# yvokeller/Show-Attend-and-Tell

Hardware: AMD Instinct MI355X
Metric: train images/sec on COCO batch=128 at 1/2/4/8 MI355X (higher is better)
Workload: dtype bf16; 1 GPU; COCO-shaped resnet152 encoder (bf16 fwd) + attention/tf/ado decoder train step, V=10000, T=27; global_batch=128, per_gpu_batch=128, seq_len=27, parallelism=dp1, hip_graph=True, encoder_decoder_overlap=True

## Files before the change

### show-attend-and-tell_amd/csrc/decoder.hip

```cpp
#include "sat_common.h"
#include "sat_internal.h"

namespace {

struct WS {
  float *mean_f, *hc0, *hc0pre, *xg, *gctx_const, *hg, *gctx, *uh_all, *gates_all, *c_in, *c_out, *h_out, *ctx_all,
      *gate_all, *fh, *fz;
  void *mean_t, *Ws, *emb_t, *h_in_t, *ctx_t, *gated_t, *hd_t, *comb_t;
  int32_t* tok;
  uint8_t* dmask;
  void *dpre_t, *dfh_t, *dfz_t, *dhg_t, *dWs_t, *dpre0_t;
  float *dcomb, *dhd, *dctx_head, *dhg, *dgated, *dh_rec, *dc, *dWs_acc, *dv_acc, *dbv_acc, *part, *demb, *dpre0,
      *colsum, *de_all;
  unsigned* ticket;
  float* gsplit;
  unsigned* gtickets;
  float* xt;
  float* fzp;
  float* am_val;
  int32_t* am_idx;
  void* emb_ws;
};
constexpr int kTicketBlocks = 16;

// ... 154 lines not shown
}

struct FGWS {
  float *dctx, *addend, *mean_term;
};
size_t carve_fg(const SatDecoderDims& d, char* base, FGWS* w) {
  const size_t B = d.B, L = d.L, D = d.D, R = B * (d.T - 1), f = 4;
  Carver c{base};
  c.take(w->dctx, R * D * f);
  if (d.attention) c.take(w->addend, B * L * D * f);
  else w->addend = nullptr;
  c.take(w->mean_term, B * D * f);
  return c.off + 256;
}

__global__ void start_tokens_kernel(int32_t* tok, int B, int T1, int start) {
  int b = blockIdx.x * blockDim.x + threadIdx.x;
  if (b < B) tok[(long)b * T1] = start;
}

__global__ void tf_prefill_kernel(const int64_t* __restrict__ caps, int B, int T, int V, int start,
                                  const uint8_t* __restrict__ keep_in, float p, const float* __restrict__ p_dev,
                                  uint64_t seed, const uint64_t* __restrict__ seed_ptr, int32_t* __restrict__ pre,
                                  uint8_t* __restrict__ keep_out) {
  const int T1 = T - 1;
  const int i = blockIdx.x * blockDim.x + threadIdx.x;
  if (i >= B * T1) return;
  const int b = i / T1, t = i - b * T1;
  bool keep = true;
  int tok = start;
  if (t > 0) {
    const int64_t c = caps[(long)b * T + t];
    tok = (c < 0 || c >= V) ? 0 : (int)c;
    if (keep_in) {
      keep = keep_in[i] != 0;
    } else {
      if (seed_ptr) seed ^= *seed_ptr * 0xD1B54A32D192ED03ULL;
      keep = sat_tf_uniform(seed, b, t) < (p_dev ? *p_dev : p);
    }
  }
  pre[i] = keep ? tok : -1;
  if (keep_out) keep_out[i] = keep ? 1 : 0;
}

struct Sampled {
  const int64_t* captions;
  float p; const float* p_dev;
  const uint8_t* mask; uint8_t* mask_out;
};
inline int32_t* tok_pre(const WS& w) { return (int32_t*)w.demb; }

template <typename T>
__global__ void ado_combine_rows_kernel(const float* fh, const float* fz, const T* emb, int rows, int E, long ld,
                                        T* comb) {
  const long n = (long)rows * E;
  for (long i = blockIdx.x * (long)blockDim.x + threadIdx.x; i < n; i += (long)gridDim.x * blockDim.x) {
    const long r = i / E;
    const int e = (int)(i - r * E);
    const long o = r * ld + e;
    comb[o] = (T)(fh[o] + fz[o] + (float)emb[o]);
  }
}

int combine_rows(const float* fh, const float* fz, const void* emb, int rows, int E, long ld, int dtype, void* comb,
                 hipStream_t s) {
  long n = (long)rows * E;
  int g = (int)((n + 255) / 256);
  if (g > 4096) g = 4096;
  if (dtype == SAT_BF16)
    hipLaunchKernelGGL(ado_combine_rows_kernel<bf16>, dim3(g), dim3(256), 0, s, fh, fz, (const bf16*)emb, rows, E, ld, (bf16*)comb);
  else
    hipLaunchKernelGGL(ado_combine_rows_kernel<float>, dim3(g), dim3(256), 0, s, fh, fz, (const float*)emb, rows, E, ld, (float*)comb);
  return (int)hipGetLastError();
}

template <typename T>
__global__ void init_state_kernel(const float* pre, int splits, long stride, int B, int E, float* hc0, T* h_t,
                                  long h_ld, float* c_in, long c_ld) {
  const long n = (long)B * 2 * E;
  for (long i = blockIdx.x * (long)blockDim.x + threadIdx.x; i < n; i += (long)gridDim.x * blockDim.x) {
    const int b = (int)(i / (2 * E)), j = (int)(i - (long)b * 2 * E);
    const float v = tanhf(sum_parts(pre, i, splits, stride));
    hc0[i] = v;
    if (j < E) h_t[(long)b * h_ld + j] = (T)v;
    else c_in[(long)b * c_ld + j - E] = v;
  }
}

struct Ctx {
  SatDecoderDims d;
  SatDecoderLayout lay;
  const float* P;
  const void* LP;
  int ts;
  long T1, R, HG;
  bool tr;
  const void* W(int64_t off) const {
    return d.dtype == SAT_BF16 ? (const void*)((const bf16*)LP + off) : (const void*)(P + off);
  }
  const float* F(int64_t off) const { return P + off; }
  void* at(void* p, long elems) const { return (char*)p + elems * ts; }
  const void* at(const void* p, long elems) const { return (const char*)p + elems * ts; }
};

int linear(const Ctx& c, int rows, int N, int K, const void* x, long ldx, const void* w, long ldw, const float* bias,
           void* y, long ldy, int y_dtype, int act, hipStream_t s, const void* add1 = nullptr, long ld_add1 = 0,
           int add1_dtype = SAT_F32, void* aux = nullptr, long ld_aux = 0, int aux_dtype = SAT_F32,
           int splits = 0, long split_stride = 0) {
  SatGemm g;
  g.partial_splits = splits; g.split_stride = split_stride;
  g.M = rows; g.N = N; g.K = K; g.dtype = c.d.dtype;
  g.A = x; g.lda = ldx; g.B = w; g.ldb = ldw;
  g.C = y; g.ldc = ldy; g.c_dtype = y_dtype; g.bias = bias; g.act = act;
  g.add1 = add1; g.ld_add1 = ld_add1; g.add1_dtype = add1_dtype;
  g.aux = aux; g.ld_aux = ld_aux; g.aux_dtype = aux_dtype;
  return sat_gemm_launch(g, s);
}

int head_forward(const Ctx& c, const WS& w, int rows, int t, bool per_step, void* preds, const uint8_t* mask_in,
                 hipStream_t s) {
  const SatDecoderDims& d = c.d;
  const int E = d.E, D = d.D, V = d.V;
  const long rs = per_step ? c.T1 : 1;
  const long oE = per_step ? (long)t * E : 0, oD = per_step ? (long)t * D : 0, oV = per_step ? (long)t * V : 0;
  if (per_step)
    SAT_CHECK((hipError_t)sat_dropout_apply(w.h_out + oE, c.T1 * E, d.B, 1, E, d.training, d.has_dropout_mask,
                                            mask_in ? mask_in + oE : nullptr, w.dmask + oE, c.T1 * E, d.seed,
                                            d.seed_ptr, t,
                                            c.at(w.hd_t, oE), c.T1 * E, d.dtype, s));
  else
    SAT_CHECK((hipError_t)sat_dropout_apply(w.h_out, E, d.B, (int)c.T1, E, d.training, d.has_dropout_mask, mask_in,
                                            w.dmask, E, d.seed, d.seed_ptr, 0, w.hd_t, E, d.dtype, s));
  if (d.ado) {
    SAT_CHECK((hipError_t)linear(c, rows, E, E, c.at(w.hd_t, oE), rs * E, c.W(c.lay.fh_w), E, c.F(c.lay.fh_b),
                                 w.fh + oE, rs * E, SAT_F32, SAT_ACT_RELU, s));
    SAT_CHECK((hipError_t)linear(c, rows, E, D, c.at(w.ctx_t, oD), rs * D, c.W(c.lay.fz_w), D, c.F(c.lay.fz_b),
                                 w.fz + oE, rs * E, SAT_F32, SAT_ACT_RELU, s));
    SAT_CHECK((hipError_t)combine_rows(w.fh + oE, w.fz + oE, c.at(w.emb_t, oE), rows, E, rs * E, d.dtype,
                                       c.at(w.comb_t, oE), s));
    SAT_CHECK((hipError_t)linear(c, rows, V, E, c.at(w.comb_t, oE), rs * E, c.W(c.lay.fout_w), E,
                                 c.F(c.lay.fout_b), c.at(preds, oV), rs * V, d.dtype, SAT_ACT_RELU, s));
  } else {
    SAT_CHECK((hipError_t)linear(c, rows, V, E, c.at(w.hd_t, oE), rs * E, c.W(c.lay.do_w), E, c.F(c.lay.do_b),
                                 c.at(preds, oV), rs * V, d.dtype, SAT_ACT_NONE, s));
  }
  return 0;
}

struct StepIO {
  const void* feats;
  float* alphas;
  const float* d_alphas;
};

int fwd_hgemm(const Ctx& c, const WS& w, const Splits& sp, int t, hipStream_t s) {
  const SatDecoderDims& d = c.d;
  const int B = d.B, D = d.D, E = d.E;
  const long T1 = c.T1, HG = c.HG;
  const void* h_t = c.at(w.h_in_t, (long)t * E);
  if (d.attention)
    return linear(c, B, (int)HG, E, h_t, T1 * E, c.W(c.lay.hcat_w), E, c.F(c.lay.hcat_b), w.hg, HG, SAT_F32,
                  SAT_ACT_NONE, s, nullptr, 0, SAT_F32, nullptr, 0, SAT_F32, sp.h, (long)B * HG);
  return linear(c, B, 4 * E, E, h_t, T1 * E, c.W(c.lay.hcat_w + (long)(E + D) * E), E, c.F(c.lay.hcat_b + E + D),
                w.hg + E + D, HG, SAT_F32, SAT_ACT_NONE, s, nullptr, 0, SAT_F32, nullptr, 0, SAT_F32, sp.h,
                (long)B * HG);
}

int fwd_attn(const Ctx& c, const WS& w, const Splits& sp, const StepIO& io, int t, hipStream_t s) {
  const SatDecoderDims& d = c.d;
  const int B = d.B, L = d.L, D = d.D, E = d.E;
  const long T1 = c.T1, HG = c.HG;
  AttnFwdArgs a{};
  a.B = B; a.L = L; a.D = D; a.E = E; a.dtype = d.dtype;
  a.Ws = w.Ws; a.uh = w.hg; a.uh_ld = HG; a.v_w = c.F(c.lay.v_w); a.v_b = c.F(c.lay.v_b); a.a = io.feats;
  a.gate_pre = w.hg + E; a.gate_ld = HG;
  a.hg_splits = sp.h; a.hg_split_stride = (long)B * HG;
  a.alpha = io.alphas + (long)t * L; a.alpha_ld = T1 * L;
  a.ctx = w.ctx_all + (long)t * D; a.ctx_ld = T1 * D;
  a.ctx_t = c.at(w.ctx_t, (long)t * D); a.ctx_t_ld = T1 * D;
  a.gate = w.gate_all + (long)t * D; a.gate_out_ld = T1 * D;
  a.gated = c.at(w.gated_t, (long)t * D); a.gated_ld = T1 * D;
  a.uh_save = w.uh_all + (long)t * E; a.uh_save_ld = T1 * E;
  return sat_attention_fwd_launch(a, s);
}

int fwd_cgemm(const Ctx& c, const WS& w, const Splits& sp, int t, hipStream_t s) {
  const SatDecoderDims& d = c.d;
  const int B = d.B, D = d.D, E = d.E;
  return linear(c, B, 4 * E, D, c.at(w.gated_t, (long)t * D), c.T1 * D, c.W(c.lay.wih + E), E + D, nullptr, w.gctx,
                4 * E, SAT_F32, SAT_ACT_NONE, s, nullptr, 0, SAT_F32, nullptr, 0, SAT_F32, sp.c, (long)B * 4 * E);
}

// ... 375 lines not shown
                         (long)B * 2 * E, B, E, w.hc0, (float*)w.h_in_t, (long)T1 * E, w.c_in, (long)T1 * E);
    SAT_LAUNCH_CHECK();
  }
  if (att) {
    SAT_CHECK((hipError_t)linear(c, B * L, E, D, img_features, D, c.W(lay->attW_w), D, c.F(lay->attW_b), w.Ws, E,
                                 d.dtype, SAT_ACT_NONE, s));
  } else {
    SAT_CHECK((hipError_t)linear(c, B, 4 * E, D, w.mean_t, D, c.W(lay->wih + E), E + D, nullptr, w.gctx_const, 4 * E,
                                 SAT_F32, SAT_ACT_NONE, s));
    SAT_CHECK((hipError_t)sat_broadcast_rows(w.mean_t, B, D, T1, d.dtype, w.gated_t, s));
    SAT_CHECK((hipError_t)sat_broadcast_rows(w.mean_t, B, D, T1, d.dtype, w.ctx_t, s));
    SAT_CHECK((hipError_t)sat_broadcast_rows(w.mean_f, B, D, T1, SAT_F32, w.ctx_all, s));
    SAT_CHECK((hipError_t)sat_fill_const(alphas, (long)B * T1 * L, 1.0f / (float)L, s));
  }
  if (d.tf)
    SAT_CHECK((hipError_t)linear(c, (int)c.R, 4 * E, E, w.emb_t, E, c.W(lay->wih), E + D, c.F(lay->bih), w.xg, 4 * E,
                                 SAT_F32, SAT_ACT_NONE, s));

  if (greedy_fused(d)) return greedy_loop(c, w, sp, io, preds, dropout_mask, tokens, s, sm);

  for (int t = 0; t < T1; ++t) {
    if (!d.tf)
      SAT_CHECK((hipError_t)linear(c, B, 4 * E, E, c.at(w.emb_t, (long)t * E), (long)T1 * E, c.W(lay->wih), E + D,
                                   c.F(lay->bih), w.xg + (long)t * 4 * E, (long)T1 * 4 * E, SAT_F32, SAT_ACT_NONE, s));
    {
      StepTimer st(d, 0, t);
      SAT_CHECK((hipError_t)fwd_hgemm(c, w, sp, t, s));
    }
    if (att) {
      {
        StepTimer st(d, 1, t);
        SAT_CHECK((hipError_t)fwd_attn(c, w, sp, io, t, s));
      }
      StepTimer st(d, 2, t);
      SAT_CHECK((hipError_t)fwd_cgemm(c, w, sp, t, s));
    }
    {
      StepTimer st(d, 3, t);
      SAT_CHECK((hipError_t)fwd_lstm(c, w, sp, t, s));
    }
    if (!d.tf) {
      SAT_CHECK((hipError_t)head_forward(c, w, B, t, true, preds, dropout_mask, s));
      if (t + 1 < T1 && sm)
        SAT_CHECK((hipError_t)sat_argmax_rows_select(c.at(preds, (long)t * d.V), d.dtype, (long)T1 * d.V, B, d.V,
                                                     w.tok + t + 1, T1, c.F(lay->embedding), E,
                                                     c.at(w.emb_t, (long)(t + 1) * E), (long)T1 * E,
                                                     tok_pre(w) + t + 1, T1, s));
      else if (t + 1 < T1)
        SAT_CHECK((hipError_t)sat_argmax_rows(c.at(preds, (long)t * d.V), d.dtype, (long)T1 * d.V, B, d.V,
                                              w.tok + t + 1, T1, c.F(lay->embedding), E,
                                              c.at(w.emb_t, (long)(t + 1) * E), (long)T1 * E, s));
    }
  }
  if (d.tf) SAT_CHECK((hipError_t)head_forward(c, w, (int)c.R, 0, false, preds, dropout_mask, s));
  if (d.training && d.seed_ptr) SAT_CHECK((hipError_t)sat_bump_seed(d.seed_ptr, s));
  if (tokens) SAT_CHECK(hipMemcpyAsync(tokens, w.tok, c.R * sizeof(int32_t), hipMemcpyDeviceToDevice, s));
  return 0;
}
}

extern "C" int sat_decoder_forward(const SatDecoderDims* dp, const SatDecoderLayout* lay, const float* params,
                                   const void* params_lp, const void* img_features, const int64_t* captions,
                                   const uint8_t* dropout_mask, void* workspace, size_t workspace_bytes, void* preds,
                                   float* alphas, int32_t* tokens, void* stream) {
  return decoder_forward(dp, lay, params, params_lp, img_features, captions, dropout_mask, workspace, workspace_bytes,
                         preds, alphas, tokens, stream, nullptr);
}

extern "C" int sat_decoder_forward_sampled(const SatDecoderDims* dp, const SatDecoderLayout* lay, const float* params,
                                           const void* params_lp, const void* img_features, const int64_t* captions,
                                           const uint8_t* dropout_mask, float tf_prob, const float* tf_prob_dev,
                                           const uint8_t* tf_mask, uint8_t* tf_mask_out, void* workspace,
                                           size_t workspace_bytes, void* preds, float* alphas, int32_t* tokens,
                                           void* stream) {
  SAT_REQUIRE(dp && dp->tf == 0);
  SAT_REQUIRE(tf_prob >= 0.f && tf_prob <= 1.f);
  const Sampled sm{captions, tf_prob, tf_prob_dev, tf_mask, tf_mask_out};
  return decoder_forward(dp, lay, params, params_lp, img_features, captions, dropout_mask, workspace, workspace_bytes,
                         preds, alphas, tokens, stream, &sm);
}

namespace {
int decoder_backward(const SatDecoderDims* dp, const SatDecoderLayout* lay, const float* params, const void* params_lp,
                     const void* img_features, void* workspace, size_t workspace_bytes, const void* preds,
                     const float* alphas, const void* d_preds, const float* d_alphas, float* grads, int accumulate,
                     int phase, void* stream, void* d_features, void* fg_workspace, size_t fg_workspace_bytes) {
  SAT_CHECK((hipError_t)check_dims(dp));
  SAT_REQUIRE(lay && params && img_features && workspace && preds && alphas && d_preds && d_alphas && grads);
  FGWS fg{};
  if (d_features && (phase & 2)) {
    SAT_REQUIRE(fg_workspace && carve_fg(*dp, nullptr, &fg) <= fg_workspace_bytes);
    SAT_REQUIRE(((uintptr_t)d_features & 15) == 0 && ((uintptr_t)fg_workspace & 15) == 0);
    carve_fg(*dp, (char*)fg_workspace, &fg);
  }
  SAT_REQUIRE((phase & 3) != 0 && phase >= 1 && phase <= 15);
  SAT_REQUIRE(dp->dtype == SAT_F32 || params_lp);
  SatPolicyScope scope(dp->policy);
  SatStampScope no_stamps(nullptr, 0);
  const SatDecoderDims& d = *dp;
  WS w;
  SAT_REQUIRE(carve(d, nullptr, &w) <= workspace_bytes);
  carve(d, (char*)workspace, &w);
  hipStream_t s = (hipStream_t)stream;
  Ctx c{d, *lay, params, params_lp, d.dtype == SAT_BF16 ? 2 : 4, d.T - 1, (long)d.B * (d.T - 1), 5L * d.E + d.D,
        use_transposed(d, *lay)};
  const int B = d.B, L = d.L, D = d.D, E = d.E, V = d.V, T1 = d.T - 1;
  const int R = (int)c.R;
  const int VP = head_ld(d);
// ... 275 lines not shown
```

### show-attend-and-tell_amd/csrc/elementwise.hip

```cpp
#include "sat_common.h"
#include "sat_internal.h"

namespace {

constexpr int kMaxGrid = 2048;
inline int grid_for(long n, int per_block = 256) {
  long g = (n + per_block - 1) / per_block;
  return (int)(g < 1 ? 1 : (g > kMaxGrid ? kMaxGrid : g));
}

template <typename T>
__global__ void nchw_to_nhwc_kernel(const float* __restrict__ x, T* __restrict__ y, int N, int C, int H, int W,
                                    int Cp) {
  long total = (long)N * H * W;
  for (long p = blockIdx.x * (long)blockDim.x + threadIdx.x; p < total; p += (long)gridDim.x * blockDim.x) {
    long n = p / ((long)H * W), hw = p - n * H * W;
    const float* src = x + n * C * H * W + hw;
    T* dst = y + p * Cp;
    if (Cp * sizeof(T) == 16) {
      uint4 u;
      T* h = (T*)&u;
#pragma unroll
      for (int c = 0; c < 16 / (int)sizeof(T); ++c) h[c] = (T)(c < C ? src[(long)c * H * W] : 0.f);
      *(uint4*)dst = u;
// ... 178 lines not shown
  for (int j = 0; j < VEC; ++j) acc[j] = 0.f;
  int l = 0;
  for (; l + 8 <= L; l += 8) {
    uint4 u[8];
#pragma unroll
    for (int k = 0; k < 8; ++k) u[k] = *(const uint4*)(p + (long)(l + k) * D);
#pragma unroll
    for (int k = 0; k < 8; ++k) {
      const T* h = (const T*)&u[k];
#pragma unroll
      for (int j = 0; j < VEC; ++j) acc[j] += (float)h[j];
    }
  }
  for (; l < L; ++l) {
    const uint4 u = *(const uint4*)(p + (long)l * D);
    const T* h = (const T*)&u;
#pragma unroll
    for (int j = 0; j < VEC; ++j) acc[j] += (float)h[j];
  }
#pragma unroll
  for (int j = 0; j < VEC; ++j) {
    const float m = acc[j] / (float)L;
    if (out_f32) out_f32[(long)b * D + d + j] = m;
    if (out_t) out_t[(long)b * D + d + j] = (T)m;
  }
}

template <typename T>
__device__ __forceinline__ void colsum_partial_body(const T* __restrict__ X, long ld, int R, int N, int rows_per,
                                                    float* __restrict__ part, int bx, int by) {
  int n = bx * 256 + (int)threadIdx.x;
  if (n >= N) return;
  int r0 = by * rows_per, r1 = min(R, r0 + rows_per);
  float s = 0.f;
  for (int r = r0; r < r1; ++r) s += (float)X[(long)r * ld + n];
  part[(long)by * N + n] = s;
}
template <typename T>
__global__ void colsum_partial_kernel(const T* __restrict__ X, long ld, int R, int N, int rows_per,
                                      float* __restrict__ part) {
  colsum_partial_body<T>(X, ld, R, N, rows_per, part, blockIdx.x, blockIdx.y);
}
template <typename T>
__device__ __forceinline__ void colsum_partial_vec_body(const T* __restrict__ X, long ld, int R, int N, int rows_per,
                                                        float* __restrict__ part, int bx, int by) {
  constexpr int VEC = 16 / sizeof(T);
  const int n = (bx * 256 + (int)threadIdx.x) * VEC;
  if (n >= N) return;
  const int r0 = by * rows_per, r1 = min(R, r0 + rows_per);
  float acc[VEC];
#pragma unroll
  for (int j = 0; j < VEC; ++j) acc[j] = 0.f;
  int r = r0;
  for (; r + 4 <= r1; r += 4) {
    uint4 u[4];
#pragma unroll
    for (int q = 0; q < 4; ++q) u[q] = *(const uint4*)(X + (long)(r + q) * ld + n);
#pragma unroll
    for (int q = 0; q < 4; ++q) {
      const T* h = (const T*)&u[q];
#pragma unroll
      for (int j = 0; j < VEC; ++j) acc[j] += (float)h[j];
    }
  }
  for (; r < r1; ++r) {
    uint4 u = *(const uint4*)(X + (long)r * ld + n);
    const T* h = (const T*)&u;
#pragma unroll
    for (int j = 0; j < VEC; ++j) acc[j] += (float)h[j];
  }
#pragma unroll
  for (int j = 0; j < VEC; ++j) part[(long)by * N + n + j] = acc[j];
}
template <typename T>
__global__ void colsum_partial_vec_kernel(const T* __restrict__ X, long ld, int R, int N, int rows_per,
                                          float* __restrict__ part) {
  colsum_partial_vec_body<T>(X, ld, R, N, rows_per, part, blockIdx.x, blockIdx.y);
}

__device__ __forceinline__ void colsum_final_body(const float* __restrict__ part, int RS, int N, int NP,
                                                  float* __restrict__ out, int accumulate, float* __restrict__ out2,
                                                  int bx) {
  int n = bx * 256 + (int)threadIdx.x;
  if (n >= N) return;
  float s0 = 0.f, s1 = 0.f, s2 = 0.f, s3 = 0.f;
  int i = 0;
  for (; i + 4 <= RS; i += 4) {
    s0 += part[(long)i * NP + n];
    s1 += part[(long)(i + 1) * NP + n];
    s2 += part[(long)(i + 2) * NP + n];
    s3 += part[(long)(i + 3) * NP + n];
  }
  for (; i < RS; ++i) s0 += part[(long)i * NP + n];
  const float s = (s0 + s1) + (s2 + s3);
  out[n] = accumulate ? out[n] + s : s;
  if (out2) out2[n] = accumulate ? out2[n] + s : s;
}
__global__ void colsum_final_kernel(const float* __restrict__ part, int RS, int N, int NP, float* __restrict__ out,
                                    int accumulate, float* __restrict__ out2) {
  colsum_final_body(part, RS, N, NP, out, accumulate, out2, blockIdx.x);
}

struct ColsumPlan {
  bool vok;
  int colblocks, RS, rows_per, np;
};
inline ColsumPlan colsum_plan(const void* X, int dtype, long ld, int R, int N, int readable = 0) {
  ColsumPlan p;
  const int vec = dtype == SAT_BF16 ? 8 : 4;
  const int nr = (N + vec - 1) / vec * vec;
  p.vok = (N % vec == 0 || (readable && nr <= ld)) && ld % vec == 0 && ((uintptr_t)X & 15) == 0;
  p.np = p.vok ? nr : N;
  p.colblocks = sat_cdiv(N, 256 * (p.vok ? vec : 1));
  int RS = 1;
  while (p.colblocks * RS < 512 && RS < 64 && (R + RS * 2 - 1) / (RS * 2) >= 16) RS *= 2;
  int rows_per = sat_cdiv(R, RS);
  RS = sat_cdiv(R, rows_per > 0 ? rows_per : 1);
  if (R <= 0) { RS = 1; rows_per = 0; }
  p.RS = RS;
  p.rows_per = rows_per;
  return p;
}

constexpr int kColsumMaxSegs = 8;
struct ColsumMultiArgs {
  int n;
  struct Seg {
    const void* X; long ld; int R, N, np, dtype, vok, colblocks, RS, rows_per, accumulate;
    int blk0, fblk0;
    float* part; float* out; float* out2;
  } seg[kColsumMaxSegs];
};
__device__ __forceinline__ int colsum_seg_of(const ColsumMultiArgs& a, int b, bool final_pass) {
  int i = 0;
  for (int k = 1; k < a.n; ++k)
    if ((final_pass ? a.seg[k].fblk0 : a.seg[k].blk0) <= b) i = k;
  return i;
}
__global__ void colsum_multi_partial_kernel(ColsumMultiArgs a) {
  const int b = blockIdx.x;
  const auto& sg = a.seg[colsum_seg_of(a, b, false)];
  const int lb = b - sg.blk0, bx = lb % sg.colblocks, by = lb / sg.colblocks;
  if (sg.vok) {
    if (sg.dtype == SAT_BF16) colsum_partial_vec_body<bf16>((const bf16*)sg.X, sg.ld, sg.R, sg.np, sg.rows_per, sg.part, bx, by);
    else colsum_partial_vec_body<float>((const float*)sg.X, sg.ld, sg.R, sg.np, sg.rows_per, sg.part, bx, by);
  } else {
    if (sg.dtype == SAT_BF16) colsum_partial_body<bf16>((const bf16*)sg.X, sg.ld, sg.R, sg.N, sg.rows_per, sg.part, bx, by);
    else colsum_partial_body<float>((const float*)sg.X, sg.ld, sg.R, sg.N, sg.rows_per, sg.part, bx, by);
  }
// ... 28 lines not shown
    } else {
      for (long i = blockIdx.x * (long)blockDim.x + threadIdx.x; i < R * C; i += stride) {
        const long r = i / C;
        p[r * ld + (i - r * C)] = 0.f;
      }
    }
  }
}

template <typename T>
__global__ void embed_gather_kernel(const float* __restrict__ W, const int32_t* __restrict__ tok, int R,
                                    long tok_stride_b, int T1, int E, T* __restrict__ out, long out_ld) {
  int r = blockIdx.x;
  if (r >= R) return;
  int b = r / T1, t = r - b * T1;
  int id = tok[(long)b * tok_stride_b + t];
  const float* src = W + (long)id * E;
  T* dst = out + (long)r * out_ld;
  for (int e = threadIdx.x; e < E; e += blockDim.x) dst[e] = (T)src[e];
}

template <typename OT>
__global__ void embed_gather_captions_kernel(const float* __restrict__ W, const int64_t* __restrict__ caps, int R,
                                             int T, int T1, int E, OT* __restrict__ out, long out_ld,
                                             int32_t* __restrict__ tok) {
  const int r = blockIdx.x;
  if (r >= R) return;
  const int b = r / T1, t = r - b * T1;
  const int id = (int)caps[(long)b * T + t];
  if (threadIdx.x == 0) tok[r] = id;
  const float* src = W + (long)id * E;
  OT* dst = out + (long)r * out_ld;
  if ((E & 3) == 0 && ((uintptr_t)src & 15) == 0) {
    for (int e = 4 * threadIdx.x; e < E; e += 4 * blockDim.x) {
      const float4 v = *(const float4*)(src + e);
      dst[e] = (OT)v.x; dst[e + 1] = (OT)v.y; dst[e + 2] = (OT)v.z; dst[e + 3] = (OT)v.w;
    }
  } else {
    for (int e = threadIdx.x; e < E; e += blockDim.x) dst[e] = (OT)src[e];
  }
}

__global__ void embed_scatter_kernel(const float* __restrict__ dX, const int32_t* __restrict__ tok, int R, int E,
                                     float* __restrict__ G) {
  int r = blockIdx.x;
  if (r >= R) return;
  int id = tok[r];
  const float* src = dX + (long)r * E;
  float* dst = G + (long)id * E;
  for (int e = threadIdx.x; e < E; e += blockDim.x) atomicAdd(dst + e, src[e]);
}

constexpr int kEmbSortMax = 16384, kEmbPiece = 32;
constexpr int kRankRows = 16, kRankParts = 16;
__global__ __launch_bounds__(256) void embed_rank_kernel(const int32_t* __restrict__ tok, int R,
                                                         int32_t* __restrict__ perm, int32_t* __restrict__ stok,
                                                         int32_t* __restrict__ seg) {
  __shared__ __attribute__((aligned(16))) int32_t st[kEmbSortMax];
  __shared__ int cnt[3][kRankParts][kRankRows];
  const int R4 = (R + 3) & ~3;
  for (int i = threadIdx.x; i < R4; i += blockDim.x) st[i] = i < R ? tok[i] : 0x7fffffff;
  __syncthreads();
  const int rl = threadIdx.x & (kRankRows - 1), part = threadIdx.x / kRankRows;
  const int r = blockIdx.x * kRankRows + rl;
  const int k = r < R ? st[r] : 0;
  const int words = R4 / 4, per = (words + kRankParts - 1) / kRankParts;
  const int w0 = part * per, w1 = min(words, w0 + per);
  int less = 0, before = 0, eq = 0;
#pragma unroll 4
  for (int wi = w0; wi < w1; ++wi) {
    const int i = 4 * wi;
    const int4 x = *(const int4*)(st + i);
    less += (x.x < k) + (x.y < k) + (x.z < k) + (x.w < k);
    eq += (x.x == k) + (x.y == k) + (x.z == k) + (x.w == k);
    before += ((x.x == k) & (i < r)) + ((x.y == k) & (i + 1 < r)) + ((x.z == k) & (i + 2 < r)) + ((x.w == k) & (i + 3 < r));
  }
  cnt[0][part][rl] = less; cnt[1][part][rl] = eq; cnt[2][part][rl] = before;
  __syncthreads();
  if (part != 0 || r >= R) return;
  for (int q = 1; q < kRankParts; ++q) { less += cnt[0][q][rl]; eq += cnt[1][q][rl]; before += cnt[2][q][rl]; }
  const int pos = less + before;
  perm[pos] = r;
  stok[pos] = k;
  seg[2 * pos] = less;
  seg[2 * pos + 1] = less + eq;
}

__global__ __launch_bounds__(64) void embed_segsum_kernel(const float* __restrict__ dX, int E,
                                                          const int32_t* __restrict__ perm,
                                                          const int32_t* __restrict__ stok,
                                                          const int32_t* __restrict__ seg, int R, float* G,
                                                          float* __restrict__ part, int accumulate) {
  const int p = blockIdx.x, e = blockIdx.y * 256 + 4 * threadIdx.x;
  const int s0 = p * kEmbPiece, n = min(R - s0, kEmbPiece);
  __shared__ int sr[kEmbPiece], stk[kEmbPiece], sa[kEmbPiece], sb[kEmbPiece];
  if ((int)threadIdx.x < n) {
    sr[threadIdx.x] = perm[s0 + threadIdx.x];
    stk[threadIdx.x] = stok[s0 + threadIdx.x];
    sa[threadIdx.x] = seg[2 * (s0 + threadIdx.x)];
    sb[threadIdx.x] = seg[2 * (s0 + threadIdx.x) + 1];
  }
  __syncthreads();
  if (e >= E) return;
  float4 x[kEmbPiece];
#pragma unroll
  for (int i = 0; i < kEmbPiece; ++i)
    x[i] = i < n ? *(const float4*)(dX + (long)sr[i] * E + e) : make_float4(0.f, 0.f, 0.f, 0.f);
  float4 acc = make_float4(0.f, 0.f, 0.f, 0.f);
  int rs = 0;
#pragma unroll
  for (int i = 0; i < kEmbPiece; ++i) {
    if (i < n) {
      acc = f4add(acc, x[i]);
      if (i + 1 == n || stk[i + 1] != stk[i]) {
        if (sa[i] == s0 + rs && sb[i] == s0 + i + 1) {
          float4* g = (float4*)(G + (long)stk[i] * E + e);
          *g = accumulate ? f4add(*g, acc) : acc;
        } else {
          *(float4*)(part + ((long)p * 2 + (rs == 0 ? 0 : 1)) * E + e) = acc;
        }
        acc = make_float4(0.f, 0.f, 0.f, 0.f);
        rs = i + 1;
      }
    }
  }
}

__global__ __launch_bounds__(256) void embed_segfix_kernel(const int32_t* __restrict__ stok,
                                                           const int32_t* __restrict__ seg, int R, int E,
                                                           const float* __restrict__ part, float* G,
                                                           int accumulate) {
  const int p = blockIdx.x, chain = threadIdx.x >> 6, e = blockIdx.y * 256 + 4 * (threadIdx.x & 63);
  const int s0 = p * kEmbPiece, s1 = min(R, s0 + kEmbPiece);
  const int sa = seg[2 * (s1 - 1)], sb = seg[2 * (s1 - 1) + 1];
  if (sb <= s1 || sa < s0) return;
  __shared__ float4 cs[3][64];
  const int p1 = (sb - 1) / kEmbPiece;
  float4 acc = make_float4(0.f, 0.f, 0.f, 0.f);
  if (e < E) {
    for (int q0 = p + 1 + chain; q0 <= p1; q0 += 32) {
      float4 y[8];
#pragma unroll
      for (int u = 0; u < 8; ++u) {
        const int q = q0 + 4 * u;
        y[u] = q <= p1 ? *(const float4*)(part + (long)q * 2 * E + e) : make_float4(0.f, 0.f, 0.f, 0.f);
      }
#pragma unroll
      for (int u = 0; u < 8; ++u) acc = f4add(acc, y[u]);
    }
  }
  if (chain > 0) cs[chain - 1][threadIdx.x & 63] = acc;
  __syncthreads();
  if (chain != 0 || e >= E) return;
  const float4 own = *(const float4*)(part + ((long)p * 2 + (sa == s0 ? 0 : 1)) * E + e);
  const float4 sum = f4add(own, f4add(f4add(acc, cs[0][threadIdx.x]), f4add(cs[1][threadIdx.x], cs[2][threadIdx.x])));
  float4* g = (float4*)(G + (long)stok[s1 - 1] * E + e);
  *g = accumulate ? f4add(*g, sum) : sum;
}

__device__ __forceinline__ bool am_better(float x, int xi, float y, int yi) { return sat_argmax_better(x, xi, y, yi); }
__device__ __forceinline__ void am_wave_reduce(float& v, int& i) {
#pragma unroll
  for (int o = 32; o > 0; o >>= 1) {
    const float ov = __shfl_xor(v, o, 64);
    const int oi = __shfl_xor(i, o, 64);
    if (am_better(ov, oi, v, i)) { v = ov; i = oi; }
  }
}
constexpr int AM_NV = 8;
template <typename T, bool VECP, bool SEL = false>
__global__ __launch_bounds__(256) void argmax_kernel(const T* __restrict__ X, long ld, int V, int32_t* __restrict__ out,
                                                     long out_stride, const float* __restrict__ emb, int E,
                                                     T* __restrict__ emb_out, long emb_ld,
                                                     const int32_t* __restrict__ pre, long pre_stride) {
  constexpr int VEC = 16 / sizeof(T);
  const int b = blockIdx.x, tid = threadIdx.x;
  int pre_tok = -1;
  if (SEL) pre_tok = pre[(long)b * pre_stride];
  const T* row = X + (long)b * ld;
  float best = -INFINITY;
  int bi = 0x7fffffff;
  if constexpr (VECP) {
    const int nvec = V / VEC;
    for (int base = 0; base < nvec; base += 256 * AM_NV) {
      uint4 u[AM_NV];
#pragma unroll
      for (int j = 0; j < AM_NV; ++j) {
        const int vi = base + j * 256 + tid;
        u[j] = vi < nvec ? *(const uint4*)(row + (long)vi * VEC) : make_uint4(0, 0, 0, 0);
      }
#pragma unroll
      for (int j = 0; j < AM_NV; ++j) {
        const int vi = base + j * 256 + tid;
        if (vi < nvec) {
          const T* h = (const T*)&u[j];
#pragma unroll
          for (int e = 0; e < VEC; ++e) {
            const float x = (float)h[e];
            if (am_better(x, vi * VEC + e, best, bi)) { best = x; bi = vi * VEC + e; }
          }
        }
      }
    }
    for (int v = nvec * VEC + tid; v < V; v += 256) {
      const float x = (float)row[v];
      if (am_better(x, v, best, bi)) { best = x; bi = v; }
    }
  } else {
    for (int v = tid; v < V; v += 256) {
// ... 149 lines not shown
  return sat_zero_segs(seg, n, s);
}
size_t sat_colsum_scratch_floats(int R, int N) { (void)R; return (size_t)64 * ((N > 0 ? N : 1) + 64); }

int sat_embed_gather(const float* W, const int32_t* tok, int B, int T1, long tok_stride_b, int E, int dtype,
                     void* out, long out_ld, hipStream_t s) {
  int R = B * T1;
  if (R <= 0) return 0;
  if (dtype == SAT_BF16)
    hipLaunchKernelGGL(embed_gather_kernel<bf16>, dim3(R), dim3(256), 0, s, W, tok, R, tok_stride_b, T1, E,
                       (bf16*)out, out_ld);
  else
    hipLaunchKernelGGL(embed_gather_kernel<float>, dim3(R), dim3(256), 0, s, W, tok, R, tok_stride_b, T1, E,
                       (float*)out, out_ld);
  return (int)hipGetLastError();
}

int sat_embed_gather_captions(const float* W, const int64_t* caps, int B, int T, int E, int dtype, void* out,
                              long out_ld, int32_t* tok, hipStream_t s) {
  const int T1 = T - 1, R = B * T1;
  if (R <= 0) return 0;
  if (dtype == SAT_BF16)
    hipLaunchKernelGGL(embed_gather_captions_kernel<bf16>, dim3(R), dim3(128), 0, s, W, caps, R, T, T1, E, (bf16*)out,
                       out_ld, tok);
  else
    hipLaunchKernelGGL(embed_gather_captions_kernel<float>, dim3(R), dim3(128), 0, s, W, caps, R, T, T1, E,
                       (float*)out, out_ld, tok);
  return (int)hipGetLastError();
}

int sat_embed_scatter_add(const float* dX, const int32_t* tok, int R, int E, float* G, hipStream_t s) {
  if (R <= 0) return 0;
  hipLaunchKernelGGL(embed_scatter_kernel, dim3(R), dim3(256), 0, s, dX, tok, R, E, G);
  return (int)hipGetLastError();
}

int sat_embed_sorted_max_rows() { return kEmbSortMax; }
static long embed_part_off(int R) { return (4L * R * 4 + 255) / 256 * 256; }
size_t sat_embed_sorted_ws_bytes(int R, int E) {
  return (size_t)(embed_part_off(R) + (long)sat_cdiv(R, kEmbPiece) * 2 * E * 4);
}
int sat_embed_scatter_add_sorted(const float* dX, const int32_t* tok, int R, int E, float* G, int accumulate, void* ws,
                                 hipStream_t s) {
  if (R <= 0) return 0;
  if (R > kEmbSortMax || E % 4 || ((uintptr_t)dX & 15) || ((uintptr_t)G & 15) || !ws) return (int)hipErrorInvalidValue;
  int32_t* perm = (int32_t*)ws;
  int32_t* stok = perm + R;
  int32_t* seg = stok + R;
  float* part = (float*)((char*)ws + embed_part_off(R));
  const int pieces = sat_cdiv(R, kEmbPiece);
  hipLaunchKernelGGL(embed_rank_kernel, dim3(sat_cdiv(R, kRankRows)), dim3(kRankRows * kRankParts), 0, s, tok, R,
                     perm, stok, seg);
  const dim3 g(pieces, sat_cdiv(E, 256));
  hipLaunchKernelGGL(embed_segsum_kernel, g, dim3(64), 0, s, dX, E, perm, stok, seg, R, G, part, accumulate);
  hipLaunchKernelGGL(embed_segfix_kernel, g, dim3(256), 0, s, stok, seg, R, E, part, G, accumulate);
  return (int)hipGetLastError();
}

int sat_argmax_rows(const void* X, int dtype, long ld, int B, int V, int32_t* out, long out_stride,
                    const float* emb, int E, void* emb_out, long emb_ld, hipStream_t s) {
  const int esz = dtype == SAT_BF16 ? 2 : 4;
  const bool vec = ((uintptr_t)X & 15) == 0 && (ld * esz) % 16 == 0;
  if (dtype == SAT_BF16) {
    if (vec) hipLaunchKernelGGL((argmax_kernel<bf16, true>), dim3(B), dim3(256), 0, s, (const bf16*)X, ld, V, out, out_stride, emb, E, (bf16*)emb_out, emb_ld, nullptr, 0);
    else hipLaunchKernelGGL((argmax_kernel<bf16, false>), dim3(B), dim3(256), 0, s, (const bf16*)X, ld, V, out, out_stride, emb, E, (bf16*)emb_out, emb_ld, nullptr, 0);
  } else {
    if (vec) hipLaunchKernelGGL((argmax_kernel<float, true>), dim3(B), dim3(256), 0, s, (const float*)X, ld, V, out, out_stride, emb, E, (float*)emb_out, emb_ld, nullptr, 0);
    else hipLaunchKernelGGL((argmax_kernel<float, false>), dim3(B), dim3(256), 0, s, (const float*)X, ld, V, out, out_stride, emb, E, (float*)emb_out, emb_ld, nullptr, 0);
  }
  return (int)hipGetLastError();
}

int sat_argmax_rows_select(const void* X, int dtype, long ld, int B, int V, int32_t* out, long out_stride,
                           const float* emb, int E, void* emb_out, long emb_ld, const int32_t* pre, long pre_stride,
                           hipStream_t s) {
  if (!pre) return (int)hipErrorInvalidValue;
  const int esz = dtype == SAT_BF16 ? 2 : 4;
  const bool vec = ((uintptr_t)X & 15) == 0 && (ld * esz) % 16 == 0;
  if (dtype == SAT_BF16) {
    if (vec) hipLaunchKernelGGL((argmax_kernel<bf16, true, true>), dim3(B), dim3(256), 0, s, (const bf16*)X, ld, V, out, out_stride, emb, E, (bf16*)emb_out, emb_ld, pre, pre_stride);
    else hipLaunchKernelGGL((argmax_kernel<bf16, false, true>), dim3(B), dim3(256), 0, s, (const bf16*)X, ld, V, out, out_stride, emb, E, (bf16*)emb_out, emb_ld, pre, pre_stride);
  } else {
    if (vec) hipLaunchKernelGGL((argmax_kernel<float, true, true>), dim3(B), dim3(256), 0, s, (const float*)X, ld, V, out, out_stride, emb, E, (float*)emb_out, emb_ld, pre, pre_stride);
    else hipLaunchKernelGGL((argmax_kernel<float, false, true>), dim3(B), dim3(256), 0, s, (const float*)X, ld, V, out, out_stride, emb, E, (float*)emb_out, emb_ld, pre, pre_stride);
  }
  return (int)hipGetLastError();
}

int sat_cast_launch(const void* x, int xd, void* y, int yd, long n, hipStream_t s) {
  if (n <= 0) return 0;
  int g = grid_for(n);
  if (xd == SAT_F32 && yd == SAT_BF16) hipLaunchKernelGGL((cast_kernel<float, bf16>), dim3(g), dim3(256), 0, s, (const float*)x, (bf16*)y, n);
  else if (xd == SAT_BF16 && yd == SAT_F32) hipLaunchKernelGGL((cast_kernel<bf16, float>), dim3(g), dim3(256), 0, s, (const bf16*)x, (float*)y, n);
  else if (xd == SAT_F32) hipLaunchKernelGGL((cast_kernel<float, float>), dim3(g), dim3(256), 0, s, (const float*)x, (float*)y, n);
  else hipLaunchKernelGGL((cast_kernel<bf16, bf16>), dim3(g), dim3(256), 0, s, (const bf16*)x, (bf16*)y, n);
  return (int)hipGetLastError();
}

extern "C" int sat_abi_version(void) { return SAT_ABI_VERSION; }

extern "C" const char* sat_error_string(int code) {
  if (code == 0) return "success";
  if (code == SAT_ERR_INVALID) return "invalid argument or unsupported shape";
  return hipGetErrorString((hipError_t)code);
}

extern "C" int sat_cast(const void* x, int x_dtype, void* y, int y_dtype, int64_t n, void* stream) {
// ... 70 lines not shown
```

Measured before the change: 20970 images/s.

## Fold seed bump into combine kernel and retune embedding-grad and colsum kernels

Moves the dropout seed increment into the ADO combine kernel when teacher forcing is on, which removes one small kernel launch. It also deepens the column-sum load unroll and rewrites the colsum final reduction with a fully unrolled register path. The embedding rank kernel now streams tokens through a chunked shared-memory buffer instead of staging the whole token array. The segmented-sum kernel uses wave ballots and readlane with float2 columns for more parallelism, and the segfix kernel hoists its loads ahead of the barrier. These are several independent micro-optimisations of small backward kernels; the chunked rank loop adds more synchronisation per chunk.

```diff
diff --git a/show-attend-and-tell_amd/csrc/decoder.hip b/show-attend-and-tell_amd/csrc/decoder.hip
--- a/show-attend-and-tell_amd/csrc/decoder.hip
+++ b/show-attend-and-tell_amd/csrc/decoder.hip
@@ -230,8 +230,9 @@
 
 template <typename T>
 __global__ void ado_combine_rows_kernel(const float* fh, const float* fz, const T* emb, int rows, int E, long ld,
-                                        T* comb) {
+                                        T* comb, uint64_t* bump) {
   const long n = (long)rows * E;
+  if (bump && blockIdx.x == 0 && threadIdx.x == 0) *bump += 1;
   for (long i = blockIdx.x * (long)blockDim.x + threadIdx.x; i < n; i += (long)gridDim.x * blockDim.x) {
     const long r = i / E;
     const int e = (int)(i - r * E);
@@ -241,14 +242,14 @@
 }
 
 int combine_rows(const float* fh, const float* fz, const void* emb, int rows, int E, long ld, int dtype, void* comb,
-                 hipStream_t s) {
+                 hipStream_t s, uint64_t* bump = nullptr) {
   long n = (long)rows * E;
   int g = (int)((n + 255) / 256);
   if (g > 4096) g = 4096;
   if (dtype == SAT_BF16)
-    hipLaunchKernelGGL(ado_combine_rows_kernel<bf16>, dim3(g), dim3(256), 0, s, fh, fz, (const bf16*)emb, rows, E, ld, (bf16*)comb);
+    hipLaunchKernelGGL(ado_combine_rows_kernel<bf16>, dim3(g), dim3(256), 0, s, fh, fz, (const bf16*)emb, rows, E, ld, (bf16*)comb, bump);
   else
-    hipLaunchKernelGGL(ado_combine_rows_kernel<float>, dim3(g), dim3(256), 0, s, fh, fz, (const float*)emb, rows, E, ld, (float*)comb);
+    hipLaunchKernelGGL(ado_combine_rows_kernel<float>, dim3(g), dim3(256), 0, s, fh, fz, (const float*)emb, rows, E, ld, (float*)comb, bump);
   return (int)hipGetLastError();
 }
 
@@ -296,7 +297,7 @@
 }
 
 int head_forward(const Ctx& c, const WS& w, int rows, int t, bool per_step, void* preds, const uint8_t* mask_in,
-                 hipStream_t s) {
+                 hipStream_t s, uint64_t* bump_seed = nullptr) {
   const SatDecoderDims& d = c.d;
   const int E = d.E, D = d.D, V = d.V;
   const long rs = per_step ? c.T1 : 1;
@@ -315,7 +316,7 @@
     SAT_CHECK((hipError_t)linear(c, rows, E, D, c.at(w.ctx_t, oD), rs * D, c.W(c.lay.fz_w), D, c.F(c.lay.fz_b),
                                  w.fz + oE, rs * E, SAT_F32, SAT_ACT_RELU, s));
     SAT_CHECK((hipError_t)combine_rows(w.fh + oE, w.fz + oE, c.at(w.emb_t, oE), rows, E, rs * E, d.dtype,
-                                       c.at(w.comb_t, oE), s));
+                                       c.at(w.comb_t, oE), s, bump_seed));
     SAT_CHECK((hipError_t)linear(c, rows, V, E, c.at(w.comb_t, oE), rs * E, c.W(c.lay.fout_w), E,
                                  c.F(c.lay.fout_b), c.at(preds, oV), rs * V, d.dtype, SAT_ACT_RELU, s));
   } else {
@@ -797,8 +798,12 @@
                                               c.at(w.emb_t, (long)(t + 1) * E), (long)T1 * E, s));
     }
   }
-  if (d.tf) SAT_CHECK((hipError_t)head_forward(c, w, (int)c.R, 0, false, preds, dropout_mask, s));
-  if (d.training && d.seed_ptr) SAT_CHECK((hipError_t)sat_bump_seed(d.seed_ptr, s));
+  const bool bump = d.training && d.seed_ptr;
+  const bool bump_in_head = bump && d.tf && d.ado;
+  if (d.tf)
+    SAT_CHECK((hipError_t)head_forward(c, w, (int)c.R, 0, false, preds, dropout_mask, s,
+                                       bump_in_head ? (uint64_t*)d.seed_ptr : nullptr));
+  if (bump && !bump_in_head) SAT_CHECK((hipError_t)sat_bump_seed(d.seed_ptr, s));
   if (tokens) SAT_CHECK(hipMemcpyAsync(tokens, w.tok, c.R * sizeof(int32_t), hipMemcpyDeviceToDevice, s));
   return 0;
 }
diff --git a/show-attend-and-tell_amd/csrc/elementwise.hip b/show-attend-and-tell_amd/csrc/elementwise.hip
--- a/show-attend-and-tell_amd/csrc/elementwise.hip
+++ b/show-attend-and-tell_amd/csrc/elementwise.hip
@@ -254,6 +254,17 @@
 #pragma unroll
   for (int j = 0; j < VEC; ++j) acc[j] = 0.f;
   int r = r0;
+  for (; r + 16 <= r1; r += 16) {
+    uint4 u[16];
+#pragma unroll
+    for (int q = 0; q < 16; ++q) u[q] = *(const uint4*)(X + (long)(r + q) * ld + n);
+#pragma unroll
+    for (int q = 0; q < 16; ++q) {
+      const T* h = (const T*)&u[q];
+#pragma unroll
+      for (int j = 0; j < VEC; ++j) acc[j] += (float)h[j];
+    }
+  }
   for (; r + 4 <= r1; r += 4) {
     uint4 u[4];
 #pragma unroll
@@ -286,17 +297,37 @@
   int n = bx * 256 + (int)threadIdx.x;
   if (n >= N) return;
   float s0 = 0.f, s1 = 0.f, s2 = 0.f, s3 = 0.f;
-  int i = 0;
-  for (; i + 4 <= RS; i += 4) {
-    s0 += part[(long)i * NP + n];
-    s1 += part[(long)(i + 1) * NP + n];
-    s2 += part[(long)(i + 2) * NP + n];
-    s3 += part[(long)(i + 3) * NP + n];
-  }
-  for (; i < RS; ++i) s0 += part[(long)i * NP + n];
+  const float o1 = accumulate ? out[n] : 0.f, o2 = accumulate && out2 ? out2[n] : 0.f;
+  constexpr int kUp = 64;
+  if (RS <= kUp) {
+    float x[kUp];
+#pragma unroll
+    for (int i = 0; i < kUp; ++i) x[i] = part[(long)min(i, RS - 1) * NP + n];
+    const int full = RS & ~3;
+#pragma unroll
+    for (int i = 0; i < kUp; ++i) {
+      if (i < full) {
+        if ((i & 3) == 0) s0 += x[i];
+        else if ((i & 3) == 1) s1 += x[i];
+        else if ((i & 3) == 2) s2 += x[i];
+        else s3 += x[i];
+      } else if (i < RS) {
+        s0 += x[i];
+      }
+    }
+  } else {
+    int i = 0;
+    for (; i + 4 <= RS; i += 4) {
+      s0 += part[(long)i * NP + n];
+      s1 += part[(long)(i + 1) * NP + n];
+      s2 += part[(long)(i + 2) * NP + n];
+      s3 += part[(long)(i + 3) * NP + n];
+    }
+    for (; i < RS; ++i) s0 += part[(long)i * NP + n];
+  }
   const float s = (s0 + s1) + (s2 + s3);
-  out[n] = accumulate ? out[n] + s : s;
-  if (out2) out2[n] = accumulate ? out2[n] + s : s;
+  out[n] = accumulate ? o1 + s : s;
+  if (out2) out2[n] = accumulate ? o2 + s : s;
 }
 __global__ void colsum_final_kernel(const float* __restrict__ part, int RS, int N, int NP, float* __restrict__ out,
                                     int accumulate, float* __restrict__ out2) {
@@ -431,28 +462,47 @@
 }
 
 constexpr int kEmbSortMax = 16384, kEmbPiece = 32;
-constexpr int kRankRows = 16, kRankParts = 16;
+constexpr int kRankRows = 16, kRankParts = 16, kRankChunk = 1024, kRankAhead = 4;
 __global__ __launch_bounds__(256) void embed_rank_kernel(const int32_t* __restrict__ tok, int R,
                                                          int32_t* __restrict__ perm, int32_t* __restrict__ stok,
                                                          int32_t* __restrict__ seg) {
-  __shared__ __attribute__((aligned(16))) int32_t st[kEmbSortMax];
+  __shared__ __attribute__((aligned(16))) int32_t st[2][kRankChunk];
   __shared__ int cnt[3][kRankParts][kRankRows];
-  const int R4 = (R + 3) & ~3;
-  for (int i = threadIdx.x; i < R4; i += blockDim.x) st[i] = i < R ? tok[i] : 0x7fffffff;
-  __syncthreads();
-  const int rl = threadIdx.x & (kRankRows - 1), part = threadIdx.x / kRankRows;
+  const __amdgpu_buffer_rsrc_t rT = sat_in_rsrc(tok, (long)R * 4);
+  const int tid = threadIdx.x, rl = tid & (kRankRows - 1), part = tid / kRankRows;
   const int r = blockIdx.x * kRankRows + rl;
-  const int k = r < R ? st[r] : 0;
-  const int words = R4 / 4, per = (words + kRankParts - 1) / kRankParts;
-  const int w0 = part * per, w1 = min(words, w0 + per);
+  const int k = (int)__builtin_amdgcn_raw_buffer_load_b32(rT, r < R ? r * 4 : (int)kSatOOB, 0, 0);
+  const int chunks = (R + kRankChunk - 1) / kRankChunk;
   int less = 0, before = 0, eq = 0;
+  for (int c0 = 0; c0 < chunks; c0 += kRankAhead) {
+    int v[kRankAhead][4];
+#pragma unroll
+    for (int u = 0; u < kRankAhead; ++u)
+#pragma unroll
+      for (int c = 0; c < 4; ++c) {
+        const int i = (c0 + u) * kRankChunk + 4 * tid + c;
+        v[u][c] = (int)__builtin_amdgcn_raw_buffer_load_b32(rT, i < R ? i * 4 : (int)kSatOOB, 0, 0);
+      }
+#pragma unroll
+    for (int u = 0; u < kRankAhead; ++u) {
+      if (c0 + u < chunks) {
+        const int base = (c0 + u) * kRankChunk;
+        int32_t* buf = st[(c0 + u) & 1];
+        const int i0 = base + 4 * tid;
+        *(int4*)(buf + 4 * tid) = make_int4(i0 < R ? v[u][0] : 0x7fffffff, i0 + 1 < R ? v[u][1] : 0x7fffffff,
+                                            i0 + 2 < R ? v[u][2] : 0x7fffffff, i0 + 3 < R ? v[u][3] : 0x7fffffff);
+        __syncthreads();
+        constexpr int per = kRankChunk / 4 / kRankParts;
 #pragma unroll 4
-  for (int wi = w0; wi < w1; ++wi) {
-    const int i = 4 * wi;
-    const int4 x = *(const int4*)(st + i);
-    less += (x.x < k) + (x.y < k) + (x.z < k) + (x.w < k);
-    eq += (x.x == k) + (x.y == k) + (x.z == k) + (x.w == k);
-    before += ((x.x == k) & (i < r)) + ((x.y == k) & (i + 1 < r)) + ((x.z == k) & (i + 2 < r)) + ((x.w == k) & (i + 3 < r));
+        for (int j = 0; j < per; ++j) {
+          const int wi = part * per + j, i = base + 4 * wi;
+          const int4 x = *(const int4*)(buf + 4 * wi);
+          less += (x.x < k) + (x.y < k) + (x.z < k) + (x.w < k);
+          eq += (x.x == k) + (x.y == k) + (x.z == k) + (x.w == k);
+          before += ((x.x == k) & (i < r)) + ((x.y == k) & (i + 1 < r)) + ((x.z == k) & (i + 2 < r)) + ((x.w == k) & (i + 3 < r));
+        }
+      }
+    }
   }
   cnt[0][part][rl] = less; cnt[1][part][rl] = eq; cnt[2][part][rl] = before;
   __syncthreads();
@@ -465,49 +515,49 @@
   seg[2 * pos + 1] = less + eq;
 }
 
+constexpr int kSegCols = 128;
+__device__ __forceinline__ float2 f2add(float2 x, float2 y) { return make_float2(x.x + y.x, x.y + y.y); }
 __global__ __launch_bounds__(64) void embed_segsum_kernel(const float* __restrict__ dX, int E,
                                                           const int32_t* __restrict__ perm,
                                                           const int32_t* __restrict__ stok,
-                                                          const int32_t* __restrict__ seg, int R, float* G,
+                                                          const int32_t* __restrict__ seg, int R, float* __restrict__ G,
                                                           float* __restrict__ part, int accumulate) {
-  const int p = blockIdx.x, e = blockIdx.y * 256 + 4 * threadIdx.x;
+  const int p = blockIdx.x, e = blockIdx.y * kSegCols + 2 * threadIdx.x;
   const int s0 = p * kEmbPiece, n = min(R - s0, kEmbPiece);
-  __shared__ int sr[kEmbPiece], stk[kEmbPiece], sa[kEmbPiece], sb[kEmbPiece];
-  if ((int)threadIdx.x < n) {
-    sr[threadIdx.x] = perm[s0 + threadIdx.x];
-    stk[threadIdx.x] = stok[s0 + threadIdx.x];
-    sa[threadIdx.x] = seg[2 * (s0 + threadIdx.x)];
-    sb[threadIdx.x] = seg[2 * (s0 + threadIdx.x) + 1];
-  }
-  __syncthreads();
-  if (e >= E) return;
-  float4 x[kEmbPiece];
-#pragma unroll
-  for (int i = 0; i < kEmbPiece; ++i)
-    x[i] = i < n ? *(const float4*)(dX + (long)sr[i] * E + e) : make_float4(0.f, 0.f, 0.f, 0.f);
-  float4 acc = make_float4(0.f, 0.f, 0.f, 0.f);
-  int rs = 0;
+  const int lane = threadIdx.x, li = min(lane, n - 1);
+  const int row = perm[s0 + li], tk = stok[s0 + li];
+  const int sa = seg[2 * (s0 + li)], sb = seg[2 * (s0 + li) + 1];
+  const int tk_next = __shfl_down(tk, 1, 64);
+  const bool end = lane < n && (lane + 1 == n || tk_next != tk);
+  const unsigned long long m_end = __ballot(end), m_whole = __ballot(end && sa >= s0 && sb == s0 + lane + 1),
+                           m_head = __ballot(end && sa <= s0);
+  const bool ok = e < E;
+  const int ec = ok ? e : 0;
+  float2 x[kEmbPiece];
 #pragma unroll
   for (int i = 0; i < kEmbPiece; ++i) {
-    if (i < n) {
-      acc = f4add(acc, x[i]);
-      if (i + 1 == n || stk[i + 1] != stk[i]) {
-        if (sa[i] == s0 + rs && sb[i] == s0 + i + 1) {
-          float4* g = (float4*)(G + (long)stk[i] * E + e);
-          *g = accumulate ? f4add(*g, acc) : acc;
-        } else {
-          *(float4*)(part + ((long)p * 2 + (rs == 0 ? 0 : 1)) * E + e) = acc;
-        }
-        acc = make_float4(0.f, 0.f, 0.f, 0.f);
-        rs = i + 1;
+    const int ri = __builtin_amdgcn_readlane(row, i);
+    x[i] = *(const float2*)(dX + (long)ri * E + ec);
+  }
+  float2 acc = make_float2(0.f, 0.f);
+#pragma unroll
+  for (int i = 0; i < kEmbPiece; ++i) {
+    acc = f2add(acc, x[i]);
+    if ((m_end >> i) & 1) {
+      if ((m_whole >> i) & 1) {
+        float2* g = (float2*)(G + (long)__builtin_amdgcn_readlane(tk, i) * E + ec);
+        if (ok) *g = accumulate ? f2add(*g, acc) : acc;
+      } else if (ok) {
+        *(float2*)(part + ((long)p * 2 + ((m_head >> i) & 1 ? 0 : 1)) * E + ec) = acc;
       }
+      acc = make_float2(0.f, 0.f);
     }
   }
 }
 
 __global__ __launch_bounds__(256) void embed_segfix_kernel(const int32_t* __restrict__ stok,
                                                            const int32_t* __restrict__ seg, int R, int E,
-                                                           const float* __restrict__ part, float* G,
+                                                           const float* __restrict__ part, float* __restrict__ G,
                                                            int accumulate) {
   const int p = blockIdx.x, chain = threadIdx.x >> 6, e = blockIdx.y * 256 + 4 * (threadIdx.x & 63);
   const int s0 = p * kEmbPiece, s1 = min(R, s0 + kEmbPiece);
@@ -515,25 +565,22 @@
   if (sb <= s1 || sa < s0) return;
   __shared__ float4 cs[3][64];
   const int p1 = (sb - 1) / kEmbPiece;
+  const int ec = e < E ? e : 0;
+  const float4 own = *(const float4*)(part + ((long)p * 2 + (sa == s0 ? 0 : 1)) * E + ec);
+  const int tk = stok[s1 - 1];
   float4 acc = make_float4(0.f, 0.f, 0.f, 0.f);
-  if (e < E) {
-    for (int q0 = p + 1 + chain; q0 <= p1; q0 += 32) {
-      float4 y[8];
-#pragma unroll
-      for (int u = 0; u < 8; ++u) {
-        const int q = q0 + 4 * u;
-        y[u] = q <= p1 ? *(const float4*)(part + (long)q * 2 * E + e) : make_float4(0.f, 0.f, 0.f, 0.f);
-      }
-#pragma unroll
-      for (int u = 0; u < 8; ++u) acc = f4add(acc, y[u]);
-    }
+  for (int q0 = p + 1 + chain; q0 <= p1; q0 += 32) {
+    float4 y[8];
+#pragma unroll
+    for (int u = 0; u < 8; ++u) y[u] = *(const float4*)(part + (long)min(q0 + 4 * u, p1) * 2 * E + ec);
+#pragma unroll
+    for (int u = 0; u < 8; ++u) acc = f4add(acc, q0 + 4 * u <= p1 ? y[u] : make_float4(0.f, 0.f, 0.f, 0.f));
   }
   if (chain > 0) cs[chain - 1][threadIdx.x & 63] = acc;
   __syncthreads();
   if (chain != 0 || e >= E) return;
-  const float4 own = *(const float4*)(part + ((long)p * 2 + (sa == s0 ? 0 : 1)) * E + e);
   const float4 sum = f4add(own, f4add(f4add(acc, cs[0][threadIdx.x]), f4add(cs[1][threadIdx.x], cs[2][threadIdx.x])));
-  float4* g = (float4*)(G + (long)stok[s1 - 1] * E + e);
+  float4* g = (float4*)(G + (long)tk * E + e);
   *g = accumulate ? f4add(*g, sum) : sum;
 }
 
@@ -789,7 +836,8 @@
   hipLaunchKernelGGL(embed_rank_kernel, dim3(sat_cdiv(R, kRankRows)), dim3(kRankRows * kRankParts), 0, s, tok, R,
                      perm, stok, seg);
   const dim3 g(pieces, sat_cdiv(E, 256));
-  hipLaunchKernelGGL(embed_segsum_kernel, g, dim3(64), 0, s, dX, E, perm, stok, seg, R, G, part, accumulate);
+  hipLaunchKernelGGL(embed_segsum_kernel, dim3(pieces, sat_cdiv(E, kSegCols)), dim3(64), 0, s, dX, E, perm, stok, seg, R,
+                     G, part, accumulate);
   hipLaunchKernelGGL(embed_segfix_kernel, g, dim3(256), 0, s, stok, seg, R, E, part, G, accumulate);
   return (int)hipGetLastError();
 }
```

Result: no change. 21070 images/s (median of 6 runs) (+0.5%).
